# joesound212985/Deepfake-Detection-using-CLIP-Based-SigLIP-2-Vision-Transformers

Measured on AMD Instinct MI355X. Metric: images/sec (train fwd+bwd) SigLIP-2-so400m@384 bf16, higher is better.
Workload: dtype bf16; 1 GPU; so400m-patch14-384 encoder+pool-head train fwd+bwd, 384x384, per-GPU batch 128, seeded random weights; global_batch=128, parallelism=dp1

## Files before the change

### deepfake-detection-using-clip-based-siglip-2-vision-transformers_amd/csrc/gemm_bf16_v2.hip

```cpp
#include <stdlib.h>
#ifdef SGL_TIMELINE
#include <stdio.h>
#include <string.h>
#endif

#include "common.hip.h"
#include "epilogue.hip.h"
#include "kernels.h"

namespace sgl {

constexpr int T_BM = 256, T_BN = 256, T_BK = 64;
constexpr int T_OP = T_BM * T_BK * 2;
constexpr int T_STAGE = 2 * T_OP;
constexpr int T_LDS = 2 * T_STAGE;
constexpr int T_CT_LD = 260;


template <int EPI, typename TOut>
__device__ __forceinline__ void store_tile256(char* smem, f32x4 (&acc)[8][4], int wr, int wc, int lane, int t, int m0,
                                              int n0, int M, int N, const EpiParams& p) {
  float* ct = reinterpret_cast<float*>(smem);
  const int g = lane >> 4, c16 = lane & 15;
  constexpr int NV = (sizeof(TOut) == 4) ? 4 : 8;
  constexpr int CPR = T_BN / NV;
  float csum[NV];
#pragma unroll
  for (int j = 0; j < NV; ++j) csum[j] = 0.f;
#define SGL_LDS_BARRIER()                                  \
  do {                                                     \
    asm volatile("s_waitcnt lgkmcnt(0)" ::: "memory");     \
    __builtin_amdgcn_s_barrier();                          \
    asm volatile("" ::: "memory");                         \
  } while (0)
  constexpr int QN = (64 * CPR) / 512;
  constexpr int RSTEP = 512 / CPR;
  const int trow = t / CPR, tcol = (t % CPR) * NV;
  const int gcol = n0 + tcol;
  const bool col_ok = gcol < N;
  constexpr bool HAS_BIAS = (EPI == EPI_BIAS_GELU || EPI == EPI_RES_F32 || EPI == EPI_QKV);
  constexpr bool FAST = HAS_BIAS || EPI == EPI_GELU_BWD;
  float bias[NV];
#pragma unroll
  for (int j = 0; j < NV; ++j) bias[j] = 0.f;
  if constexpr (HAS_BIAS) {
    if (col_ok) Vec<float, NV>::ld(p.bias + gcol, bias);
  }
  size_t qkv_c0 = 0;
  int qkv_pad = 0;
  if constexpr (EPI == EPI_QKV) {
    const int dm = p.heads * p.head_dim;
    const int which = gcol / dm;
    const int hc = gcol - which * dm;
    const int h = hc / p.head_dim;
    const int d = hc - h * p.head_dim;
    qkv_c0 = ((size_t)which * p.batch * p.heads + h) * (size_t)p.tokens * p.head_dim_pad + d;
    qkv_pad = (d + NV == p.head_dim) ? (p.head_dim_pad - p.head_dim) / NV : 0;
  }
  using PreT = u32x4;
  constexpr bool HAS_PRE = (EPI == EPI_RES_F32 || EPI == EPI_GELU_BWD);
  PreT pre[2][QN];
  auto load_pre = [&](int pass, PreT (&dst)[QN]) {
    if constexpr (HAS_PRE) {
#pragma unroll
      for (int q = 0; q < QN; ++q) {
        const int row = trow + q * RSTEP;
        const int grow = m0 + (row >> 5) * 128 + pass * 32 + (row & 31);
        const void* src = (EPI == EPI_RES_F32)
                              ? (const void*)(p.res + (size_t)grow * p.ldr + gcol)
                              : (const void*)(reinterpret_cast<const TOut*>(p.aux) + (size_t)grow * p.ldaux + gcol);
        dst[q] = (grow < M && col_ok) ? *reinterpret_cast<const PreT*>(src) : PreT{0u, 0u, 0u, 0u};
      }
    }
  };
  load_pre(0, pre[0]);
#pragma unroll
  for (int pass = 0; pass < 4; ++pass) {
    if (pass + 1 < 4) load_pre(pass + 1, pre[(pass + 1) & 1]);
    if (pass == 0) __syncthreads(); else SGL_LDS_BARRIER();
#pragma unroll
    for (int i2 = 0; i2 < 2; ++i2)
#pragma unroll
      for (int j = 0; j < 4; ++j)
#pragma unroll
        for (int r = 0; r < 4; ++r)
          ct[(wr * 32 + i2 * 16 + g * 4 + r) * T_CT_LD + wc * 64 + j * 16 + c16] = acc[2 * pass + i2][j][r];
    SGL_LDS_BARRIER();
#define SGL_CT_GROW(q) (m0 + ((q) >> 5) * 128 + pass * 32 + ((q) & 31))
    if constexpr (EPI == EPI_F32) {
      if (p.atomic) {
        float* outp = reinterpret_cast<float*>(p.out);
        const int w = t >> 6;
#pragma unroll 2
        for (int rr = 0; rr < 8; ++rr) {
          const int row = w + rr * 8;
          const int grow = SGL_CT_GROW(row);
          if (grow >= M) continue;
#pragma unroll
          for (int h = 0; h < 4; ++h) {
            const int col = lane + 64 * h;
            if (n0 + col < N) atomicAdd(outp + (size_t)grow * p.ldo + n0 + col, ct[row * T_CT_LD + col] * p.alpha);
          }
        }
        continue;
      }
    }
#pragma unroll
    for (int q = 0; q < QN; ++q) {
      const int row = trow + q * RSTEP;
      const int grow = SGL_CT_GROW(row);
      if (grow < M && col_ok) {
        float v[NV];
        Vec<float, NV>::ld(ct + row * T_CT_LD + tcol, v);
        if constexpr (EPI == EPI_RES_F32) {
          const f32x4 r = __builtin_bit_cast(f32x4, pre[pass & 1][q]);
#pragma unroll
          for (int j = 0; j < NV; ++j) v[j] = r[j] + (v[j] + bias[j]);
          Vec<float, NV>::st_nt(reinterpret_cast<float*>(p.out) + (size_t)grow * p.ldo + gcol, v);
        } else if constexpr (EPI == EPI_BIAS_GELU) {
          float a[NV];
          if (p.out && p.gelu_grad_form) {
#pragma unroll
            for (int j = 0; j < NV; ++j) gelu_tanh_both(v[j] + bias[j], a[j], v[j]);
          } else {
#pragma unroll
            for (int j = 0; j < NV; ++j) {
              v[j] += bias[j];
              a[j] = gelu_tanh(v[j]);
            }
          }
          if (p.out) Vec<TOut, NV>::st_nt(reinterpret_cast<TOut*>(p.out) + (size_t)grow * p.ldo + gcol, v);
          Vec<TOut, NV>::st_nt(reinterpret_cast<TOut*>(p.out2) + (size_t)grow * p.ldo2 + gcol, a);
        } else if constexpr (EPI == EPI_QKV) {
          int b = (int)((float)grow * __builtin_amdgcn_rcpf((float)p.tokens));
          int n = grow - b * p.tokens;
          if (n < 0) { b -= 1; n += p.tokens; }
          else if (n >= p.tokens) { b += 1; n -= p.tokens; }
#pragma unroll
          for (int j = 0; j < NV; ++j) v[j] += bias[j];
          TOut* dst = reinterpret_cast<TOut*>(p.out) + qkv_c0 + ((size_t)b * p.heads * p.tokens + n) * p.head_dim_pad;
          Vec<TOut, NV>::st_nt(dst, v);
          if (qkv_pad) {
            float z[NV];
#pragma unroll
            for (int j = 0; j < NV; ++j) z[j] = 0.f;
            for (int k = 1; k <= qkv_pad; ++k) Vec<TOut, NV>::st_nt(dst + k * NV, z);
          }
        } else if constexpr (EPI == EPI_GELU_BWD) {
          float u[NV];
          if constexpr (NV == 8) {
            const lo_x8<TOut> ub = __builtin_bit_cast(lo_x8<TOut>, pre[pass & 1][q]);
#pragma unroll
            for (int j = 0; j < NV; ++j) u[j] = (float)ub[j];
          } else {
            const f32x4 uf = __builtin_bit_cast(f32x4, pre[pass & 1][q]);
#pragma unroll
            for (int j = 0; j < NV; ++j) u[j] = uf[j];
          }
          if (p.gelu_grad_form) {
#pragma unroll
            for (int j = 0; j < NV; ++j) v[j] *= u[j];
          } else {
#pragma unroll
            for (int j = 0; j < NV; ++j) v[j] *= gelu_tanh_grad(u[j]);
          }
          Vec<TOut, NV>::st_nt(reinterpret_cast<TOut*>(p.out) + (size_t)grow * p.ldo + gcol, v);
#pragma unroll
          for (int j = 0; j < NV; ++j) csum[j] += v[j];
        } else {
          epi_apply<EPI, TOut, NV>(p, grow, gcol, N, v);
        }
      }
    }
  }
#undef SGL_CT_GROW
  if constexpr (EPI == EPI_GELU_BWD) {
    if (p.colsum) {
      SGL_LDS_BARRIER();
      constexpr int GROUPS = 512 / CPR;
#pragma unroll
      for (int j = 0; j < NV; ++j) ct[(t / CPR) * T_BN + (t % CPR) * NV + j] = csum[j];
      SGL_LDS_BARRIER();
      if (t < T_BN && n0 + t < N) {
        float s = 0.f;
#pragma unroll
        for (int gI = 0; gI < GROUPS; ++gI) s += ct[gI * T_BN + t];
        if (p.colsum_ld > 0)
          p.colsum[(size_t)(m0 >> 7) * p.colsum_ld + n0 + t] = s;
        else
          atomicAdd(p.colsum + n0 + t, s);
      }
    }
  }
}

__device__ __forceinline__ int unit_of_block(int bid, int per) { return (bid & 7) * per + (bid >> 3); }

__device__ __forceinline__ void tile_of_unit(int u, int tiles_m, int tiles_n, int& tile_m, int& tile_n, int bh = 8) {
  const int band = u / (bh * tiles_n);
  const int rows = (tiles_m - band * bh < bh) ? tiles_m - band * bh : bh;
  const int r = u - band * bh * tiles_n;
  tile_n = r / rows;
  tile_m = band * bh + (r - tile_n * rows);
}

__device__ __forceinline__ bool tile_of_local(int xcd, int v, int tiles_m, int tiles_n, int cgw, int& tm, int& tn) {
  const int r_lo = (xcd * tiles_m) >> 3, r_hi = ((xcd + 1) * tiles_m) >> 3;
  const int R = r_hi - r_lo;
  if (v >= R * tiles_n) return false;
  const int full = R * cgw;
  const int g = v / full, rem = v - g * full;
  const int w = (tiles_n - g * cgw < cgw) ? tiles_n - g * cgw : cgw;
  const int r = rem / w;
  tm = r_lo + r;
  tn = g * cgw + (rem - r * w);
  return true;
}

__device__ __forceinline__ void pp_dma16(u32x4 desc, uint32_t lds_addr, uint32_t voff) {
  asm volatile("s_mov_b32 m0, %0\n\ts_nop 0\n\tbuffer_load_dwordx4 %1, %2, 0 offen lds"
               :: "s"(lds_addr), "v"(voff), "s"(desc) : "memory");
}
__device__ __forceinline__ u32x4 pp_desc(const void* base, uint32_t bytes) {
  const uint64_t q = (uint64_t)base;
  u32x4 d = {(uint32_t)q, (uint32_t)(q >> 32) & 0xffffu, bytes, 0x00020000u};
  return d;
}
#define SGL_PP_END_READ8()                                              \
  do {                                                                  \
    asm volatile("s_waitcnt vmcnt(8) lgkmcnt(0)" ::: "memory");         \
    __builtin_amdgcn_sched_barrier(0);                                  \
    __builtin_amdgcn_s_barrier();                                       \
    __builtin_amdgcn_sched_barrier(0);                                  \
  } while (0)
#define SGL_PP_END_MFMA()                 \
  do {                                    \
    __builtin_amdgcn_sched_barrier(0);    \
    __builtin_amdgcn_s_barrier();         \
    __builtin_amdgcn_sched_barrier(0);    \
  } while (0)

#ifdef SGL_TIMELINE
__device__ unsigned long long g_nt6_tl[4];
__device__ unsigned long long g_tn6_tl[12];
#define SGL_TL_STAMP(v) const unsigned long long v = __builtin_readcyclecounter()
#else
#define SGL_TL_STAMP(v)
#endif
template <int EPI, typename TOut, typename TIn>
__global__ __launch_bounds__(512, 2) void gemm_nt6_kernel(const TIn* __restrict__ A, int lda,
                                                          const TIn* __restrict__ B, int ldb, int M, int N, int K,
                                                          int tiles_m, int tiles_n, int band_h, EpiParams p) {
  extern __shared__ __attribute__((aligned(16))) char smem[];
  SGL_TL_STAMP(tl0);
  const int ntiles = tiles_m * tiles_n;
  int tile_m, tile_n;
  if (band_h < 0) {
    if (!tile_of_local(blockIdx.x & 7, blockIdx.x >> 3, tiles_m, tiles_n, -band_h, tile_m, tile_n)) return;
  } else {
    const int unit = unit_of_block(blockIdx.x, (ntiles + 7) >> 3);
    if (unit >= ntiles) return;
    tile_of_unit(unit, tiles_m, tiles_n, tile_m, tile_n, band_h);
  }
  const int t = threadIdx.x, lane = t & 63;
  const int w = __builtin_amdgcn_readfirstlane(t >> 6);
  const int wr = (w >> 1) & 1, wc = (w & 1) + 2 * (w >> 2), grp = w >> 2;
  const int m0 = tile_m * T_BM, n0 = tile_n * T_BN;
  const int rows_a = (M - m0 < T_BM) ? M - m0 : T_BM;
  const int rows_b = (N - n0 < T_BN) ? N - n0 : T_BN;
  const u32x4 da = pp_desc(A + (size_t)m0 * lda, (uint32_t)(((size_t)(rows_a - 1) * lda + K) * 2));
  const u32x4 db = pp_desc(B + (size_t)n0 * ldb, (uint32_t)(((size_t)(rows_b - 1) * ldb + K) * 2));
  const uint32_t lds0 = (uint32_t)(size_t)((SGL_LDS char*)smem);

  const int drow = lane >> 3, dchunk = (lane & 7) ^ drow;
  uint32_t voff[4][2], ldst[4][2];
#pragma unroll
  for (int u = 0; u < 4; ++u)
#pragma unroll
    for (int q = 0; q < 2; ++q) {
      const int ul = 16 * w + 8 * q;
      int r0;
      if (u == 0) r0 = (ul < 64) ? ul : ul + 64;
      else if (u == 3) r0 = (ul < 64) ? ul + 64 : ul + 128;
      else r0 = (ul >> 5) * 64 + (ul & 31) + (u == 2 ? 32 : 0);
      const int row = r0 + drow;
      const bool isA = (u == 0 || u == 3);
      const int lim = isA ? rows_a : rows_b;
      const int ld = isA ? lda : ldb;
      voff[u][q] = (row < lim) ? (uint32_t)(row * ld + dchunk * 8) * 2u : SGL_OOB;
      ldst[u][q] = lds0 + (isA ? 0 : T_OP) + (uint32_t)r0 * 128u;
    }
  const int nk = (K + T_BK - 1) / T_BK;
  auto issue = [&](int u, int kt) {
    const int k0 = kt * T_BK;
    const bool kok = (kt < nk) && (k0 + dchunk * 8 < K);
    const uint32_t sb = (uint32_t)((kt & 1) * T_STAGE);
    const u32x4 d = (u == 0 || u == 3) ? da : db;
#pragma unroll
    for (int q = 0; q < 2; ++q)
      pp_dma16(d, ldst[u][q] + sb, (kok && voff[u][q] != SGL_OOB) ? voff[u][q] + (uint32_t)k0 * 2u : SGL_OOB);
  };

  const int frow = lane & 15, fg = lane >> 4, fsw = frow & 7;
  const uint32_t fa_base = (uint32_t)((wr * 128 + frow) * 128);
  const uint32_t fb_base = (uint32_t)(T_OP + (wc * 64 + frow) * 128);
  const uint32_t c0 = (uint32_t)(((0 + fg) ^ fsw) << 4), c1 = (uint32_t)(((4 + fg) ^ fsw) << 4);
  const bool active = (n0 + wc * 64 < N) && (m0 + wr * 128 < M);

  f32x4 acc[8][4];
#pragma unroll
  for (int i = 0; i < 8; ++i)
#pragma unroll
    for (int j = 0; j < 4; ++j) acc[i][j] = f32x4{0.f, 0.f, 0.f, 0.f};

  issue(0, 0); issue(1, 0); issue(2, 0); issue(3, 0);
  issue(0, 1); issue(1, 1); issue(2, 1);
  SGL_PP_END_READ8();
  if (grp == 1) SGL_PP_END_MFMA();

  lo_x8<TIn> fa[8], fb[8];
  for (int kt = 0; kt < nk; ++kt) {
    const char* base = smem + (kt & 1) * T_STAGE;
    const char* pa = base + fa_base;
    const char* pb = base + fb_base;
    if (active) {
#pragma unroll
      for (int f = 0; f < 8; ++f) fb[f] = *reinterpret_cast<const lo_x8<TIn>*>(pb + (f & 3) * 2048 + ((f >> 2) ? c1 : c0));
#pragma unroll
      for (int f = 0; f < 8; ++f) fa[f] = *reinterpret_cast<const lo_x8<TIn>*>(pa + (f & 3) * 2048 + ((f >> 2) ? c1 : c0));
    }
    issue(3, kt + 1);
    SGL_PP_END_READ8();
    if (active) {
      __builtin_amdgcn_s_setprio(1);
#pragma unroll
      for (int h = 0; h < 2; ++h)
#pragma unroll
        for (int i = 0; i < 4; ++i)
#pragma unroll
          for (int j = 0; j < 4; ++j)
            acc[i][j] = mfma_16x16x32(fa[4 * h + i], fb[4 * h + j], acc[i][j]);
      __builtin_amdgcn_s_setprio(0);
    }
    SGL_PP_END_MFMA();
    if (active) {
#pragma unroll
      for (int f = 0; f < 8; ++f) fa[f] = *reinterpret_cast<const lo_x8<TIn>*>(pa + (4 + (f & 3)) * 2048 + ((f >> 2) ? c1 : c0));
    }
    issue(0, kt + 2); issue(1, kt + 2); issue(2, kt + 2);
    SGL_PP_END_READ8();
    if (active) {
      __builtin_amdgcn_s_setprio(1);
#pragma unroll
      for (int h = 0; h < 2; ++h)
#pragma unroll
        for (int i = 0; i < 4; ++i)
#pragma unroll
          for (int j = 0; j < 4; ++j)
            acc[4 + i][j] = mfma_16x16x32(fa[4 * h + i], fb[4 * h + j], acc[4 + i][j]);
      __builtin_amdgcn_s_setprio(0);
    }
    SGL_PP_END_MFMA();
  }
  if (grp == 0) SGL_PP_END_MFMA();
  asm volatile("s_waitcnt vmcnt(0)" ::: "memory");
#ifdef SGL_TIMELINE
  if (p.atomic == 77) return;
#endif
  SGL_TL_STAMP(tl1);
  store_tile256<EPI, TOut>(smem, acc, wr, wc, lane, t, m0, n0, M, N, p);
#ifdef SGL_TIMELINE
  SGL_TL_STAMP(tl2);
  if (t == 0) {
    atomicAdd(&g_nt6_tl[0], tl1 - tl0);
    atomicAdd(&g_nt6_tl[1], tl2 - tl1);
    atomicAdd(&g_nt6_tl[2], 1ull);
  }
#endif
}

template <typename TIn>
__global__ __launch_bounds__(512, 2) void gemm_tn6_kernel(const TIn* __restrict__ A, int lda,
                                                          const TIn* __restrict__ B, int ldb, int Mred, int N1, int N2,
                                                          int m_per_split, int nsplits, int tiles_1, int tiles_2,
                                                          EpiParams p) {
  extern __shared__ __attribute__((aligned(16))) char smem[];
  const int ntiles = tiles_1 * tiles_2;
  const int nunits = ntiles * nsplits;
  const int unit = unit_of_block(blockIdx.x, (nunits + 7) >> 3);
  if (unit >= nunits) return;
  const int split = unit / ntiles, trem = unit - split * ntiles;
  const int tile1 = trem / tiles_2, tile2 = trem - tile1 * tiles_2;
  const int t = threadIdx.x, lane = t & 63;
  const int w = __builtin_amdgcn_readfirstlane(t >> 6);
  const int wr = (w >> 1) & 1, wc = (w & 1) + 2 * (w >> 2), grp = w >> 2;
  const int n1_0 = tile1 * T_BM, n2_0 = tile2 * T_BN;
  const int m_begin = split * m_per_split;
  const int m_end = (m_begin + m_per_split < Mred) ? m_begin + m_per_split : Mred;
  const int rows = m_end - m_begin;
  const u32x4 da = pp_desc(A + (size_t)m_begin * lda, (uint32_t)((size_t)rows * lda * 2));
  const u32x4 db = pp_desc(B + (size_t)m_begin * ldb, (uint32_t)((size_t)rows * ldb * 2));
  const uint32_t lds0 = (uint32_t)(size_t)((SGL_LDS char*)smem);

  const int dr2 = lane >> 5, dslot = lane & 31;
  uint32_t voff[4][2], ldst[4][2];
#pragma unroll
  for (int u = 0; u < 4; ++u)
#pragma unroll
    for (int q = 0; q < 2; ++q) {
      const int r0 = 32 * (u >> 1) + 4 * w + 2 * q;
      const int row = r0 + dr2;
      const int chunk = dslot ^ (2 * (row & 3) + 8 * ((row >> 3) & 1));
      const bool isA = (u & 1) == 0;
      const int col = (isA ? n1_0 : n2_0) + chunk * 8;
      const int lim = isA ? N1 : N2;
      const int ld = isA ? lda : ldb;
      voff[u][q] = (col < lim) ? (uint32_t)(row * ld + col) * 2u : SGL_OOB;
      ldst[u][q] = lds0 + (isA ? 0 : T_OP) + (uint32_t)r0 * 512u;
    }
  auto issue = [&](int u, int kt) {
    const uint32_t r0 = (uint32_t)kt * T_BK;
    const uint32_t sb = (uint32_t)((kt & 1) * T_STAGE);
    const bool isA = (u & 1) == 0;
    const u32x4 d = isA ? da : db;
    const uint32_t adv = r0 * (uint32_t)(isA ? lda : ldb) * 2u;
#pragma unroll
    for (int q = 0; q < 2; ++q) pp_dma16(d, ldst[u][q] + sb, voff[u][q] == SGL_OOB ? SGL_OOB : voff[u][q] + adv);
  };

  const int fg = lane >> 4, fq = (lane >> 2) & 3, fp = lane & 3;
  const uint32_t swz = (uint32_t)(32 * fq + 128 * (fg & 1));
  const uint32_t frow = (uint32_t)((8 * fg + fq) * 512);
  const uint32_t fa_col = ((uint32_t)(wr * 256 + 8 * fp)) ^ swz;
  const uint32_t fb_col = ((uint32_t)(wc * 128 + 8 * fp)) ^ swz;
  const bool active = (n2_0 + wc * 64 < N2) && (n1_0 + wr * 128 < N1);

  f32x4 acc[8][4];
#pragma unroll
  for (int i = 0; i < 8; ++i)
#pragma unroll
    for (int j = 0; j < 4; ++j) acc[i][j] = f32x4{0.f, 0.f, 0.f, 0.f};

  const int nk = (rows + T_BK - 1) / T_BK;
  issue(0, 0); issue(1, 0); issue(2, 0); issue(3, 0);
  issue(0, 1); issue(1, 1);
  SGL_PP_END_READ8();
  if (grp == 1) SGL_PP_END_MFMA();

#define SGL_TR6(ptr) \
  __builtin_shufflevector(lds_read_tr16<TIn>(ptr), lds_read_tr16<TIn>((ptr) + 4 * 512), 0, 1, 2, 3, 4, 5, 6, 7)
  lo_x8<TIn> fa[8], fb[4];
#ifdef SGL_TIMELINE
  unsigned long long tlp[5] = {0, 0, 0, 0, 0};
#define SGL_TLP(i) do { const unsigned long long n_ = __builtin_readcyclecounter(); tlp[i] += n_ - tl_last; tl_last = n_; } while (0)
  unsigned long long tl_last = __builtin_readcyclecounter();
#else
#define SGL_TLP(i)
#endif
  for (int kt = 0; kt < nk; ++kt) {
    const char* base = smem + (kt & 1) * T_STAGE + frow;
#pragma unroll
    for (int h = 0; h < 2; ++h) {
      if (active) {
#pragma unroll
        for (int j = 0; j < 4; ++j) fb[j] = SGL_TR6(base + T_OP + h * 32 * 512 + (fb_col ^ (uint32_t)(j * 32)));
#pragma unroll
        for (int i = 0; i < 8; ++i) fa[i] = SGL_TR6(base + h * 32 * 512 + (fa_col ^ (uint32_t)(i * 32)));
      }
      if (h == 0) { issue(2, kt + 1); issue(3, kt + 1); }
      else { issue(0, kt + 2); issue(1, kt + 2); }
#ifdef SGL_TIMELINE
      SGL_TLP(0);
      asm volatile("s_waitcnt vmcnt(8) lgkmcnt(0)" ::: "memory");
      SGL_TLP(1);
      __builtin_amdgcn_sched_barrier(0);
      __builtin_amdgcn_s_barrier();
      __builtin_amdgcn_sched_barrier(0);
      SGL_TLP(2);
#else
      SGL_PP_END_READ8();
#endif
      if (active) {
        __builtin_amdgcn_s_setprio(1);
#pragma unroll
        for (int i = 0; i < 8; ++i)
#pragma unroll
          for (int j = 0; j < 4; ++j)
            acc[i][j] = mfma_16x16x32(fa[i], fb[j], acc[i][j]);
        __builtin_amdgcn_s_setprio(0);
      }
#ifdef SGL_TIMELINE
      asm volatile("s_nop 0" ::"v"(acc[0][0]), "v"(acc[7][3]));
      SGL_TLP(3);
#endif
      SGL_PP_END_MFMA();
      SGL_TLP(4);
    }
  }
#ifdef SGL_TIMELINE
  if (lane == 0 && active && (w == 0 || w == 4)) {
    for (int i = 0; i < 5; ++i) atomicAdd(&g_tn6_tl[(w >> 2) * 6 + i], tlp[i]);
    atomicAdd(&g_tn6_tl[(w >> 2) * 6 + 5], (unsigned long long)(2 * nk));
  }
#endif
#undef SGL_TR6
  if (grp == 0) SGL_PP_END_MFMA();
  asm volatile("s_waitcnt vmcnt(0)" ::: "memory");
  EpiParams pq = p;
  if (p.split_stride) pq.out = reinterpret_cast<float*>(p.out) + (size_t)split * p.split_stride;
  store_tile256<EPI_F32, float>(smem, acc, wr, wc, lane, t, n1_0, n2_0, N1, N2, pq);
}

template <int EPI, typename TOut, typename TIn>
static hipError_t launch_nt256(const TIn* A, int lda, const TIn* B, int ldb, int M, int N, int K, const EpiParams& p,
                               hipStream_t s) {
  const hipError_t e = set_max_dynamic_lds_once<&gemm_nt6_kernel<EPI, TOut, TIn>>(T_LDS);
  if (e != hipSuccess) return e;
  const int tiles_m = (M + T_BM - 1) / T_BM, tiles_n = (N + T_BN - 1) / T_BN;
  static const int band_env = getenv("SGL_BAND") ? atoi(getenv("SGL_BAND")) : 0;
  const int band_h = band_env != 0 ? band_env : -8;
  const int grid = band_h < 0 ? 8 * (((tiles_m + 7) / 8) * tiles_n)
                              : ((tiles_m * tiles_n + 7) / 8) * 8;
  EpiParams pp = p;
#ifdef SGL_TIMELINE
  static const bool skip_epi = getenv("SGL_NT6_SKIP_EPI") != nullptr;
  if (skip_epi && EPI != EPI_F32) pp.atomic = 77;
#endif
  hipLaunchKernelGGL((gemm_nt6_kernel<EPI, TOut, TIn>), dim3(grid), dim3(512), T_LDS, s, A, lda, B, ldb, M, N, K, tiles_m,
                     tiles_n, band_h, pp);
#ifdef SGL_TIMELINE
  if (getenv("SGL_TIMELINE")) {
    unsigned long long h[4];
    (void)hipStreamSynchronize(s);
    (void)hipMemcpyFromSymbol(h, HIP_SYMBOL(g_nt6_tl), sizeof(h));
    if (h[2])
      fprintf(stderr, "[timeline] gemm_nt6 EPI %d M=%d N=%d K=%d: %llu tiles, main loop %.0f, epilogue %.0f cycles per tile\n", EPI, M,
              N, K, h[2], (double)h[0] / h[2], (double)h[1] / h[2]);
    memset(h, 0, sizeof(h));
    (void)hipMemcpyToSymbol(HIP_SYMBOL(g_nt6_tl), h, sizeof(h));
  }
#endif
  return hipGetLastError();
}

template <typename TIn>
static hipError_t gemm_nt256(const void* A, int lda, const void* B, int ldb, int M, int N, int K, int epi, int out_dtype,
                             const EpiParams& p, hipStream_t s) {
  return dispatch_epilogue<TIn>(epi, out_dtype, [&](auto tag) {
    using T = decltype(tag);
    return launch_nt256<T::epi, typename T::out, TIn>((const TIn*)A, lda, (const TIn*)B, ldb, M, N, K, p, s);
  });
}
hipError_t gemm_nt256_bf16(const void* A, int lda, const void* B, int ldb, int M, int N, int K, int epi, int out_dtype,
                           const EpiParams& p, hipStream_t s) {
  return gemm_nt256<bf16>(A, lda, B, ldb, M, N, K, epi, out_dtype, p, s);
}
hipError_t gemm_nt256_f16(const void* A, int lda, const void* B, int ldb, int M, int N, int K, int epi, int out_dtype,
                          const EpiParams& p, hipStream_t s) {
  return gemm_nt256<f16>(A, lda, B, ldb, M, N, K, epi, out_dtype, p, s);
}

template <typename TIn>
static hipError_t gemm_tn256(const void* A, int lda, const void* B, int ldb, int Mred, int N1, int N2, int m_per,
                             int splits, const EpiParams& p, hipStream_t s) {
  const hipError_t e = set_max_dynamic_lds_once<&gemm_tn6_kernel<TIn>>(T_LDS);
  if (e != hipSuccess) return e;
  const int tiles_1 = (N1 + T_BM - 1) / T_BM, tiles_2 = (N2 + T_BN - 1) / T_BN;
  const int grid = ((tiles_1 * tiles_2 * splits + 7) / 8) * 8;
  hipLaunchKernelGGL(gemm_tn6_kernel<TIn>, dim3(grid), dim3(512), T_LDS, s, (const TIn*)A, lda, (const TIn*)B, ldb, Mred,
                     N1, N2, m_per, splits, tiles_1, tiles_2, p);
#ifdef SGL_TIMELINE
  if (getenv("SGL_TIMELINE")) {
    unsigned long long h[12];
    (void)hipStreamSynchronize(s);
    (void)hipMemcpyFromSymbol(h, HIP_SYMBOL(g_tn6_tl), sizeof(h));
    for (int g = 0; g < 2; ++g)
      if (h[g * 6 + 5])
        fprintf(stderr, "[timeline] gemm_tn6 N1=%d N2=%d Mred=%d splits=%d group %d, cycles per slot pair (read slot + MFMA slot): issue "
                "reads+DMA %.0f, wait %.0f, barrier %.0f, 32 MFMAs %.0f, barrier %.0f\n", N1, N2, Mred, splits, g,
                (double)h[g * 6 + 0] / h[g * 6 + 5], (double)h[g * 6 + 1] / h[g * 6 + 5], (double)h[g * 6 + 2] / h[g * 6 + 5],
                (double)h[g * 6 + 3] / h[g * 6 + 5], (double)h[g * 6 + 4] / h[g * 6 + 5]);
    memset(h, 0, sizeof(h));
    (void)hipMemcpyToSymbol(HIP_SYMBOL(g_tn6_tl), h, sizeof(h));
  }
#endif
  return hipGetLastError();
}

hipError_t gemm_tn256_bf16(const void* A, int lda, const void* B, int ldb, int Mred, int N1, int N2, int m_per,
                           int splits, const EpiParams& p, hipStream_t s) {
  return gemm_tn256<bf16>(A, lda, B, ldb, Mred, N1, N2, m_per, splits, p, s);
}
hipError_t gemm_tn256_f16(const void* A, int lda, const void* B, int ldb, int Mred, int N1, int N2, int m_per,
                          int splits, const EpiParams& p, hipStream_t s) {
  return gemm_tn256<f16>(A, lda, B, ldb, Mred, N1, N2, m_per, splits, p, s);
}

}
```

Measured before the change: 434.4 images/sec.

## Use tall 512x128 tiles for ragged last column in NT GEMM

When the last N tile column is at most 128 wide, the NT GEMM now pairs two 256-row tiles into one 512x128 tall tile. This avoids wasting half of a 256x256 tile on out-of-range columns. The change adds a tile-geometry template, a new tile-map header that accounts for the merged units, and a larger LDS allocation for the epilogue types that can use tall tiles. The larger LDS request may cut occupancy for those kernels, and the mixed tile shapes make scheduling harder.

```diff
diff --git a/deepfake-detection-using-clip-based-siglip-2-vision-transformers_amd/csrc/gemm_bf16_v2.hip b/deepfake-detection-using-clip-based-siglip-2-vision-transformers_amd/csrc/gemm_bf16_v2.hip
--- a/deepfake-detection-using-clip-based-siglip-2-vision-transformers_amd/csrc/gemm_bf16_v2.hip
+++ b/deepfake-detection-using-clip-based-siglip-2-vision-transformers_amd/csrc/gemm_bf16_v2.hip
@@ -7,6 +7,7 @@
 #include "common.hip.h"
 #include "epilogue.hip.h"
 #include "kernels.h"
+#include "nt_tile_map.h"
 
 namespace sgl {
 
@@ -14,16 +15,31 @@
 constexpr int T_OP = T_BM * T_BK * 2;
 constexpr int T_STAGE = 2 * T_OP;
 constexpr int T_LDS = 2 * T_STAGE;
-constexpr int T_CT_LD = 260;
-
-
-template <int EPI, typename TOut>
+constexpr int T_CT_PAD = 4;
+
+template <bool TALL>
+struct NtGeom {
+  static constexpr int BM = TALL ? 512 : T_BM, BN = TALL ? 128 : T_BN;
+  static constexpr int WR = BM / 128;
+  static constexpr int OPA = BM * T_BK * 2;
+  static constexpr int STAGE = OPA + BN * T_BK * 2;
+  static constexpr int NU = STAGE / 16384;
+};
+constexpr int NT_LDS_TALL = 2 * NtGeom<true>::STAGE;
+static_assert(NtGeom<false>::STAGE == T_STAGE && NtGeom<false>::OPA == T_OP, "the square geometry is the shared one");
+template <int EPI>
+constexpr bool kNtTallEpi = (EPI == EPI_STORE || EPI == EPI_RES_F32 || EPI == EPI_QKV);
+
+
+template <int EPI, typename TOut, int BN = T_BN, int WR = 2>
 __device__ __forceinline__ void store_tile256(char* smem, f32x4 (&acc)[8][4], int wr, int wc, int lane, int t, int m0,
                                               int n0, int M, int N, const EpiParams& p) {
+  static_assert(BN == T_BN || kNtTallEpi<EPI>, "this epilogue has no tall-tile form");
+  constexpr int T_CT_LD = BN + T_CT_PAD;
   float* ct = reinterpret_cast<float*>(smem);
   const int g = lane >> 4, c16 = lane & 15;
   constexpr int NV = (sizeof(TOut) == 4) ? 4 : 8;
-  constexpr int CPR = T_BN / NV;
+  constexpr int CPR = BN / NV;
   float csum[NV];
 #pragma unroll
   for (int j = 0; j < NV; ++j) csum[j] = 0.f;
@@ -33,7 +49,7 @@
     __builtin_amdgcn_s_barrier();                          \
     asm volatile("" ::: "memory");                         \
   } while (0)
-  constexpr int QN = (64 * CPR) / 512;
+  constexpr int QN = (32 * WR * CPR) / 512;
   constexpr int RSTEP = 512 / CPR;
   const int trow = t / CPR, tcol = (t % CPR) * NV;
   const int gcol = n0 + tcol;
@@ -194,29 +210,6 @@
   }
 }
 
-__device__ __forceinline__ int unit_of_block(int bid, int per) { return (bid & 7) * per + (bid >> 3); }
-
-__device__ __forceinline__ void tile_of_unit(int u, int tiles_m, int tiles_n, int& tile_m, int& tile_n, int bh = 8) {
-  const int band = u / (bh * tiles_n);
-  const int rows = (tiles_m - band * bh < bh) ? tiles_m - band * bh : bh;
-  const int r = u - band * bh * tiles_n;
-  tile_n = r / rows;
-  tile_m = band * bh + (r - tile_n * rows);
-}
-
-__device__ __forceinline__ bool tile_of_local(int xcd, int v, int tiles_m, int tiles_n, int cgw, int& tm, int& tn) {
-  const int r_lo = (xcd * tiles_m) >> 3, r_hi = ((xcd + 1) * tiles_m) >> 3;
-  const int R = r_hi - r_lo;
-  if (v >= R * tiles_n) return false;
-  const int full = R * cgw;
-  const int g = v / full, rem = v - g * full;
-  const int w = (tiles_n - g * cgw < cgw) ? tiles_n - g * cgw : cgw;
-  const int r = rem / w;
-  tm = r_lo + r;
-  tn = g * cgw + (rem - r * w);
-  return true;
-}
-
 __device__ __forceinline__ void pp_dma16(u32x4 desc, uint32_t lds_addr, uint32_t voff) {
   asm volatile("s_mov_b32 m0, %0\n\ts_nop 0\n\tbuffer_load_dwordx4 %1, %2, 0 offen lds"
                :: "s"(lds_addr), "v"(voff), "s"(desc) : "memory");
@@ -229,6 +222,13 @@
 #define SGL_PP_END_READ8()                                              \
   do {                                                                  \
     asm volatile("s_waitcnt vmcnt(8) lgkmcnt(0)" ::: "memory");         \
+    __builtin_amdgcn_sched_barrier(0);                                  \
+    __builtin_amdgcn_s_barrier();                                       \
+    __builtin_amdgcn_sched_barrier(0);                                  \
+  } while (0)
+#define SGL_PP_END_READ10()                                             \
+  do {                                                                  \
+    asm volatile("s_waitcnt vmcnt(10) lgkmcnt(0)" ::: "memory");        \
     __builtin_amdgcn_sched_barrier(0);                                  \
     __builtin_amdgcn_s_barrier();                                       \
     __builtin_amdgcn_sched_barrier(0);                                  \
@@ -247,63 +247,67 @@
 #else
 #define SGL_TL_STAMP(v)
 #endif
-template <int EPI, typename TOut, typename TIn>
-__global__ __launch_bounds__(512, 2) void gemm_nt6_kernel(const TIn* __restrict__ A, int lda,
-                                                          const TIn* __restrict__ B, int ldb, int M, int N, int K,
-                                                          int tiles_m, int tiles_n, int band_h, EpiParams p) {
-  extern __shared__ __attribute__((aligned(16))) char smem[];
+template <int EPI, typename TOut, typename TIn, bool TALL>
+__device__ __forceinline__ void nt6_tile(char* smem, const TIn* __restrict__ A, int lda, const TIn* __restrict__ B,
+                                         int ldb, int M, int N, int K, int tile_m, int tile_n, const EpiParams& p) {
+  using G = NtGeom<TALL>;
   SGL_TL_STAMP(tl0);
-  const int ntiles = tiles_m * tiles_n;
-  int tile_m, tile_n;
-  if (band_h < 0) {
-    if (!tile_of_local(blockIdx.x & 7, blockIdx.x >> 3, tiles_m, tiles_n, -band_h, tile_m, tile_n)) return;
-  } else {
-    const int unit = unit_of_block(blockIdx.x, (ntiles + 7) >> 3);
-    if (unit >= ntiles) return;
-    tile_of_unit(unit, tiles_m, tiles_n, tile_m, tile_n, band_h);
-  }
   const int t = threadIdx.x, lane = t & 63;
   const int w = __builtin_amdgcn_readfirstlane(t >> 6);
-  const int wr = (w >> 1) & 1, wc = (w & 1) + 2 * (w >> 2), grp = w >> 2;
+  const int wr = TALL ? (w & 3) : (w >> 1) & 1, wc = TALL ? (w >> 2) : (w & 1) + 2 * (w >> 2), grp = w >> 2;
   const int m0 = tile_m * T_BM, n0 = tile_n * T_BN;
-  const int rows_a = (M - m0 < T_BM) ? M - m0 : T_BM;
-  const int rows_b = (N - n0 < T_BN) ? N - n0 : T_BN;
+  const int rows_a = (M - m0 < G::BM) ? M - m0 : G::BM;
+  const int rows_b = (N - n0 < G::BN) ? N - n0 : G::BN;
   const u32x4 da = pp_desc(A + (size_t)m0 * lda, (uint32_t)(((size_t)(rows_a - 1) * lda + K) * 2));
   const u32x4 db = pp_desc(B + (size_t)n0 * ldb, (uint32_t)(((size_t)(rows_b - 1) * ldb + K) * 2));
   const uint32_t lds0 = (uint32_t)(size_t)((SGL_LDS char*)smem);
 
+  auto unit_is_a = [](int u) { return TALL ? (u != 2) : (u == 0 || u == 3); };
   const int drow = lane >> 3, dchunk = (lane & 7) ^ drow;
-  uint32_t voff[4][2], ldst[4][2];
-#pragma unroll
-  for (int u = 0; u < 4; ++u)
+  uint32_t voff[G::NU][2], ldst[G::NU][2];
+#pragma unroll
+  for (int u = 0; u < G::NU; ++u)
 #pragma unroll
     for (int q = 0; q < 2; ++q) {
       const int ul = 16 * w + 8 * q;
       int r0;
-      if (u == 0) r0 = (ul < 64) ? ul : ul + 64;
-      else if (u == 3) r0 = (ul < 64) ? ul + 64 : ul + 128;
-      else r0 = (ul >> 5) * 64 + (ul & 31) + (u == 2 ? 32 : 0);
+      if constexpr (TALL) {
+        if (u == 2) r0 = ul;
+        else r0 = ((ul < 64) ? ul : ul + 64) + (u >= 3 ? 64 : 0) + ((u == 1 || u == 4) ? 256 : 0);
+      } else {
+        if (u == 0) r0 = (ul < 64) ? ul : ul + 64;
+        else if (u == 3) r0 = (ul < 64) ? ul + 64 : ul + 128;
+        else r0 = (ul >> 5) * 64 + (ul & 31) + (u == 2 ? 32 : 0);
+      }
       const int row = r0 + drow;
-      const bool isA = (u == 0 || u == 3);
+      const bool isA = unit_is_a(u);
       const int lim = isA ? rows_a : rows_b;
       const int ld = isA ? lda : ldb;
       voff[u][q] = (row < lim) ? (uint32_t)(row * ld + dchunk * 8) * 2u : SGL_OOB;
-      ldst[u][q] = lds0 + (isA ? 0 : T_OP) + (uint32_t)r0 * 128u;
+      ldst[u][q] = lds0 + (isA ? 0 : G::OPA) + (uint32_t)r0 * 128u;
     }
   const int nk = (K + T_BK - 1) / T_BK;
   auto issue = [&](int u, int kt) {
     const int k0 = kt * T_BK;
     const bool kok = (kt < nk) && (k0 + dchunk * 8 < K);
-    const uint32_t sb = (uint32_t)((kt & 1) * T_STAGE);
-    const u32x4 d = (u == 0 || u == 3) ? da : db;
+    const uint32_t sb = (uint32_t)((kt & 1) * G::STAGE);
+    const u32x4 d = unit_is_a(u) ? da : db;
 #pragma unroll
     for (int q = 0; q < 2; ++q)
       pp_dma16(d, ldst[u][q] + sb, (kok && voff[u][q] != SGL_OOB) ? voff[u][q] + (uint32_t)k0 * 2u : SGL_OOB);
   };
+  auto issue_first = [&](int kt) { issue(0, kt); issue(1, kt); issue(2, kt); };
+  auto issue_second = [&](int kt) {
+    issue(3, kt);
+    if constexpr (TALL) issue(4, kt);
+  };
+  auto end_read = [&]() {
+    if constexpr (TALL) SGL_PP_END_READ10(); else SGL_PP_END_READ8();
+  };
 
   const int frow = lane & 15, fg = lane >> 4, fsw = frow & 7;
   const uint32_t fa_base = (uint32_t)((wr * 128 + frow) * 128);
-  const uint32_t fb_base = (uint32_t)(T_OP + (wc * 64 + frow) * 128);
+  const uint32_t fb_base = (uint32_t)(G::OPA + (wc * 64 + frow) * 128);
   const uint32_t c0 = (uint32_t)(((0 + fg) ^ fsw) << 4), c1 = (uint32_t)(((4 + fg) ^ fsw) << 4);
   const bool active = (n0 + wc * 64 < N) && (m0 + wr * 128 < M);
 
@@ -313,14 +317,14 @@
 #pragma unroll
     for (int j = 0; j < 4; ++j) acc[i][j] = f32x4{0.f, 0.f, 0.f, 0.f};
 
-  issue(0, 0); issue(1, 0); issue(2, 0); issue(3, 0);
-  issue(0, 1); issue(1, 1); issue(2, 1);
-  SGL_PP_END_READ8();
+  issue_first(0); issue_second(0);
+  issue_first(1);
+  end_read();
   if (grp == 1) SGL_PP_END_MFMA();
 
   lo_x8<TIn> fa[8], fb[8];
   for (int kt = 0; kt < nk; ++kt) {
-    const char* base = smem + (kt & 1) * T_STAGE;
+    const char* base = smem + (kt & 1) * G::STAGE;
     const char* pa = base + fa_base;
     const char* pb = base + fb_base;
     if (active) {
@@ -329,8 +333,8 @@
 #pragma unroll
       for (int f = 0; f < 8; ++f) fa[f] = *reinterpret_cast<const lo_x8<TIn>*>(pa + (f & 3) * 2048 + ((f >> 2) ? c1 : c0));
     }
-    issue(3, kt + 1);
-    SGL_PP_END_READ8();
+    issue_second(kt + 1);
+    end_read();
     if (active) {
       __builtin_amdgcn_s_setprio(1);
 #pragma unroll
@@ -347,8 +351,8 @@
 #pragma unroll
       for (int f = 0; f < 8; ++f) fa[f] = *reinterpret_cast<const lo_x8<TIn>*>(pa + (4 + (f & 3)) * 2048 + ((f >> 2) ? c1 : c0));
     }
-    issue(0, kt + 2); issue(1, kt + 2); issue(2, kt + 2);
-    SGL_PP_END_READ8();
+    issue_first(kt + 2);
+    end_read();
     if (active) {
       __builtin_amdgcn_s_setprio(1);
 #pragma unroll
@@ -368,7 +372,7 @@
   if (p.atomic == 77) return;
 #endif
   SGL_TL_STAMP(tl1);
-  store_tile256<EPI, TOut>(smem, acc, wr, wc, lane, t, m0, n0, M, N, p);
+  store_tile256<EPI, TOut, G::BN, G::WR>(smem, acc, wr, wc, lane, t, m0, n0, M, N, p);
 #ifdef SGL_TIMELINE
   SGL_TL_STAMP(tl2);
   if (t == 0) {
@@ -377,6 +381,24 @@
     atomicAdd(&g_nt6_tl[2], 1ull);
   }
 #endif
+}
+
+template <int EPI, typename TOut, typename TIn>
+__global__ __launch_bounds__(512, 2) void gemm_nt6_kernel(const TIn* __restrict__ A, int lda,
+                                                          const TIn* __restrict__ B, int ldb, int M, int N, int K,
+                                                          int tiles_m, int tiles_n, int band_h, int tall_last,
+                                                          EpiParams p) {
+  extern __shared__ __attribute__((aligned(16))) char smem[];
+  NtUnit unit;
+  if (!nt_unit_of_block(blockIdx.x, tiles_m, tiles_n, band_h, tall_last, unit)) return;
+  const int tile_m = __builtin_amdgcn_readfirstlane(unit.tile_m), tile_n = __builtin_amdgcn_readfirstlane(unit.tile_n);
+  if constexpr (kNtTallEpi<EPI>) {
+    if (__builtin_amdgcn_readfirstlane(unit.tall)) {
+      nt6_tile<EPI, TOut, TIn, true>(smem, A, lda, B, ldb, M, N, K, tile_m, tile_n, p);
+      return;
+    }
+  }
+  nt6_tile<EPI, TOut, TIn, false>(smem, A, lda, B, ldb, M, N, K, tile_m, tile_n, p);
 }
 
 template <typename TIn>
@@ -514,20 +536,23 @@
 template <int EPI, typename TOut, typename TIn>
 static hipError_t launch_nt256(const TIn* A, int lda, const TIn* B, int ldb, int M, int N, int K, const EpiParams& p,
                                hipStream_t s) {
-  const hipError_t e = set_max_dynamic_lds_once<&gemm_nt6_kernel<EPI, TOut, TIn>>(T_LDS);
+  const hipError_t e = set_max_dynamic_lds_once<&gemm_nt6_kernel<EPI, TOut, TIn>>(kNtTallEpi<EPI> ? NT_LDS_TALL : T_LDS);
   if (e != hipSuccess) return e;
   const int tiles_m = (M + T_BM - 1) / T_BM, tiles_n = (N + T_BN - 1) / T_BN;
+  static const bool tall_env = !(getenv("SGL_TALL") && atoi(getenv("SGL_TALL")) == 0);
+  const int n_last = N - (tiles_n - 1) * T_BN;
+  const int tall_last = (kNtTallEpi<EPI> && tall_env && n_last <= NtGeom<true>::BN && tiles_m >= 2) ? 1 : 0;
+  const int lds_bytes = tall_last ? NT_LDS_TALL : T_LDS;
   static const int band_env = getenv("SGL_BAND") ? atoi(getenv("SGL_BAND")) : 0;
   const int band_h = band_env != 0 ? band_env : -8;
-  const int grid = band_h < 0 ? 8 * (((tiles_m + 7) / 8) * tiles_n)
-                              : ((tiles_m * tiles_n + 7) / 8) * 8;
+  const int grid = nt_grid(tiles_m, tiles_n, band_h, tall_last);
   EpiParams pp = p;
 #ifdef SGL_TIMELINE
   static const bool skip_epi = getenv("SGL_NT6_SKIP_EPI") != nullptr;
   if (skip_epi && EPI != EPI_F32) pp.atomic = 77;
 #endif
-  hipLaunchKernelGGL((gemm_nt6_kernel<EPI, TOut, TIn>), dim3(grid), dim3(512), T_LDS, s, A, lda, B, ldb, M, N, K, tiles_m,
-                     tiles_n, band_h, pp);
+  hipLaunchKernelGGL((gemm_nt6_kernel<EPI, TOut, TIn>), dim3(grid), dim3(512), lds_bytes, s, A, lda, B, ldb, M, N, K,
+                     tiles_m, tiles_n, band_h, tall_last, pp);
 #ifdef SGL_TIMELINE
   if (getenv("SGL_TIMELINE")) {
     unsigned long long h[4];
diff --git a/deepfake-detection-using-clip-based-siglip-2-vision-transformers_amd/csrc/nt_tile_map.h b/deepfake-detection-using-clip-based-siglip-2-vision-transformers_amd/csrc/nt_tile_map.h
--- /dev/null
+++ b/deepfake-detection-using-clip-based-siglip-2-vision-transformers_amd/csrc/nt_tile_map.h
@@ -0,0 +1,88 @@
+#pragma once
+
+#if defined(__HIPCC__)
+#define SGL_HD __host__ __device__ __forceinline__
+#else
+#define SGL_HD inline
+#endif
+
+namespace sgl {
+
+struct NtUnit {
+  int tile_m, tile_n;
+  int tall;
+};
+
+SGL_HD int unit_of_block(int bid, int per) { return (bid & 7) * per + (bid >> 3); }
+
+SGL_HD int nt_last_col_units(int rows, int tall_last) { return tall_last ? (rows + 1) >> 1 : rows; }
+
+SGL_HD int nt_band_units(int rows, int tiles_n, int tall_last) {
+  return rows * (tiles_n - 1) + nt_last_col_units(rows, tall_last);
+}
+SGL_HD int nt_grouped_units(int tiles_m, int tiles_n, int bh, int tall_last) {
+  return (tiles_m / bh) * nt_band_units(bh, tiles_n, tall_last) + nt_band_units(tiles_m % bh, tiles_n, tall_last);
+}
+SGL_HD bool nt_unit_grouped(int u, int tiles_m, int tiles_n, int bh, int tall_last, NtUnit& o) {
+  if (u >= nt_grouped_units(tiles_m, tiles_n, bh, tall_last)) return false;
+  const int per_band = nt_band_units(bh, tiles_n, tall_last);
+  const int band = u / per_band;
+  const int rows = (tiles_m - band * bh < bh) ? tiles_m - band * bh : bh;
+  const int r = u - band * per_band;
+  const int sq = rows * (tiles_n - 1);
+  if (r < sq) {
+    o.tile_n = r / rows;
+    o.tile_m = band * bh + (r - o.tile_n * rows);
+    o.tall = 0;
+  } else {
+    const int k = r - sq;
+    o.tile_n = tiles_n - 1;
+    o.tile_m = band * bh + (tall_last ? 2 * k : k);
+    o.tall = (tall_last && 2 * k + 1 < rows) ? 1 : 0;
+  }
+  return true;
+}
+
+SGL_HD int nt_local_units(int R, int tiles_n, int tall_last) { return R * (tiles_n - 1) + nt_last_col_units(R, tall_last); }
+SGL_HD bool nt_unit_local(int xcd, int v, int tiles_m, int tiles_n, int cgw, int tall_last, NtUnit& o) {
+  const int r_lo = (xcd * tiles_m) >> 3, r_hi = ((xcd + 1) * tiles_m) >> 3;
+  const int R = r_hi - r_lo;
+  if (v >= nt_local_units(R, tiles_n, tall_last)) return false;
+  const int full = R * cgw;
+  const int groups = (tiles_n + cgw - 1) / cgw;
+  int g = v / full;
+  if (g > groups - 1) g = groups - 1;
+  const int rem = v - g * full;
+  const int w = (tiles_n - g * cgw < cgw) ? tiles_n - g * cgw : cgw;
+  o.tall = 0;
+  if (!tall_last || g != groups - 1) {
+    const int r = rem / w;
+    o.tile_m = r_lo + r;
+    o.tile_n = g * cgw + (rem - r * w);
+    return true;
+  }
+  const int wf = w - 1;
+  const int per_pair = 2 * wf + 1;
+  const int pr = rem / per_pair, q = rem - pr * per_pair;
+  if (q < 2 * wf && 2 * pr + (q >= wf) < R) {
+    o.tile_m = r_lo + 2 * pr + (q >= wf);
+    o.tile_n = g * cgw + (q >= wf ? q - wf : q);
+    return true;
+  }
+  o.tile_m = r_lo + 2 * pr;
+  o.tile_n = tiles_n - 1;
+  o.tall = (2 * pr + 1 < R) ? 1 : 0;
+  return true;
+}
+
+SGL_HD int nt_grid(int tiles_m, int tiles_n, int band_h, int tall_last) {
+  if (band_h < 0) return 8 * nt_local_units((tiles_m + 7) >> 3, tiles_n, tall_last);
+  return ((nt_grouped_units(tiles_m, tiles_n, band_h, tall_last) + 7) >> 3) << 3;
+}
+SGL_HD bool nt_unit_of_block(int bid, int tiles_m, int tiles_n, int band_h, int tall_last, NtUnit& o) {
+  if (band_h < 0) return nt_unit_local(bid & 7, bid >> 3, tiles_m, tiles_n, -band_h, tall_last, o);
+  const int total = nt_grouped_units(tiles_m, tiles_n, band_h, tall_last);
+  return nt_unit_grouped(unit_of_block(bid, (total + 7) >> 3), tiles_m, tiles_n, band_h, tall_last, o);
+}
+
+}
```

Measured after the change: 437.7 images/sec (median of 6 runs). About the same (+0.8%).
